# oval-group/GNN_branching

Measured on NVIDIA B200. Metric: gnn_subdomains_scored_per_sec, higher is better.
Workload: dtype fp16x3 (fp32 accumulate)

## Files before the change

### gnn_branching_b200/csrc/gnnb_tc.cu

```cuda
#include "gnnb_prop_body.cuh"
#include "gnnb_umma.cuh"

namespace gnnb {
namespace {

using namespace tcx;

constexpr uint32_t ACOL = 0, DCOL = 64, WG_COLS = 128;

struct WG {
    uint32_t land;
    uint32_t mbar_mma, mbar_tma;
    uint32_t ph_mma, ph_tma;
    uint32_t tmem;
    uint32_t tmem0;
    uint32_t acol;
    int t;
    int bar_threads;
    int wg;
    bool lead_warp;
};

__device__ __forceinline__ void wg_barrier(const WG& c) { named_bar(1 + c.wg, c.bar_threads); }

// ... 878 lines not shown
#pragma unroll
                        for (int i = 0; i < 16; ++i) o[i] = relu_nan(fmaf(node_ >= 0 ? l_ : 0.f, wl[i], fmaf(node_ >= 0 ? u_ : 0.f, wu[i], o[i])));
                        uint32_t w[16];
                        split16(o, w);
                        tmem_st16(c.tmem + D + 64 + 16 * qd, w);
                    }
                }
                gemm_sync(c);
                if (c.lead_warp) {
                    tc_fence_after();
                    if (elect_one()) {
                        WG c2 = c;
                        c2.acol = D + 64;
                        issue_ts(c, W + INF_WN, W + INF_WN + WPLANE, 64, D, false);
                        issue_ts(c2, W + INF_WI, W + INF_WI + WPLANE, 64, D, true);
                        umma_commit(c.mbar_mma);
                    }
                    __syncwarp();
                }
            } else {
                gemm_ts_start(c, W + UPD_W3, W + UPD_W3 + 2 * WPLANE, 128, D);
            }
            return true;
        };
        bool have = cur.valid() ? start_item(cur, 0, node_n, l_n, u_n) : false;
        for (; cur.valid(); cur.next(), cur1.next(), cur2.next(), ++it) {
            const uint32_t buf = it & 1u;
            const uint32_t acc_empty = smem_u32(&tl->acc_empty[buf]);
            const int dom = cur.pair * PD + j;
            const int node = node_n;
            const float l = l_n, u = u_n;
            const int slot0 = slot0_n;
            fetch_bounds(cur1, node_nn);
            node_nn = fetch_node(cur2);
            auto advance = [&]() { have = cur1.valid() ? start_item(cur1, it + 1, node_n, l_n, u_n) : false; };
            if (!have) {
                advance();
                continue;
            }
            const int64_t tile = (int64_t)dom * ntiles + cur.tile;
#ifdef GNNB_TRACE
            c0_ = clock64(); ++c_tiles;
#endif
            const Ratio q = compute_ratio(l, u);
            const float gate = (q.r0 != 0.0f) ? 1.0f : 0.0f;
            const bool amb = (q.amb != 0.0f) && node >= 0;
            const unsigned bal = __ballot_sync(0xffffffffu, amb);
            if ((c.t & 31) == 0) tl->wcnt[j * 2 + h][c.t >> 5] = __popc(bal);
            unsigned char* img = a.mu_out ? reinterpret_cast<unsigned char*>(a.mu_out) + tile * (int64_t)ABUF : nullptr;
            if (inp) {
                gemm_finish(c);
                if (h == 0 && c.t == 0) mbar_arrive(acc_empty);
                c.acol = D + 64;
                CTR(1);
                {
                    float v0[16], v1[16];
                    tmem_ld32_sync(c.tmem + D + h * 32, v0, v1);
#pragma unroll
                    for (int qq = 0; qq < 2; ++qq) {
                        float (&v)[16] = qq ? v1 : v0;
                        const int qd = Q0 + qq;
                        float bb[16];
                        lds16(tl->bias[0] + qd * 16, bb);
#pragma unroll
                        for (int i = 0; i < 16; ++i) v[i] = relu_nan(v[i] + bb[i]);
                        a_store16(c, qd, v);
                    }
                }
                CTR(2);
                gemm_ts_start(c, W + INF_B22, W + INF_B22 + WPLANE, 64, D);
                gemm_finish(c);
                CTR(3);
                bad |= nan_watch(a.nan_doms, dom, epilogue_to_mu_pair<false>(c, h, pair_bar, D, tl->bias[1], 1.0f, node >= 0, img, stage, advance));
                CTR(6);
                continue;
            }
            gemm_finish(c);
            if (h == 0 && c.t == 0) mbar_arrive(acc_empty);
            c.acol = D + 64;
            CTR(1);
#pragma unroll
            for (int qq = 0; qq < 2; ++qq) {
                const int qd = Q0 + qq;
                float x[16], y[16], bb[16];
                {
                    uint32_t ra[16], rb[16];
                    tmem_ld16(c.tmem + D + qd * 16, ra);
                    tmem_ld16(c.tmem + D + 64 + qd * 16, rb);
                    tmem_wait16(ra, x);
                    tmem_wait16(rb, y);
                }
                lds16(tl->bias[0] + qd * 16, bb);
#pragma unroll
                for (int i = 0; i < 16; ++i) x[i] = relu_nan(fmaf(q.r0, x[i], fmaf(q.r1, y[i], bb[i])));
                a_store16(c, qd, x);
            }
            CTR(2);
            gemm_ts_start(c, W + UPD_WC, W + UPD_WC + WPLANE, 64, D);
            int slot = slot0 + __popc(bal & ((1u << (c.t & 31)) - 1u));
#pragma unroll
            for (int w = 0; w < 3; ++w) slot += (w < (c.t >> 5)) ? tl->wcnt[j * 2 + h][w] : 0;
            const float* rt = rlx + (size_t)(slot >> 7) * (TILE * P) + (size_t)(slot & (TILE - 1)) * 4 + (size_t)(8 * h) * (TILE * 4);
            float4 rx[8];
#pragma unroll
            for (int i = 0; i < 8; ++i) rx[i] = amb ? ldg4_now(rt + (size_t)i * (TILE * 4)) : make_float4(0.f, 0.f, 0.f, 0.f);
            gemm_finish(c);
            CTR(3);
            {
                float v0[16], v1[16];
                tmem_ld32_sync(c.tmem + D + h * 32, v0, v1);
#pragma unroll
                for (int qq = 0; qq < 2; ++qq) {
                    float (&v)[16] = qq ? v1 : v0;
                    const int qd = Q0 + qq;
                    float bb[16];
                    lds16(tl->bias[1] + qd * 16, bb);
#pragma unroll
                    for (int hh = 0; hh < 4; ++hh) {
                        const float4 x = rx[qq * 4 + hh];
                        v[hh * 4 + 0] = relu_nan(v[hh * 4 + 0] + x.x + bb[hh * 4 + 0]);
                        v[hh * 4 + 1] = relu_nan(v[hh * 4 + 1] + x.y + bb[hh * 4 + 1]);
                        v[hh * 4 + 2] = relu_nan(v[hh * 4 + 2] + x.z + bb[hh * 4 + 2]);
                        v[hh * 4 + 3] = relu_nan(v[hh * 4 + 3] + x.w + bb[hh * 4 + 3]);
                    }
                    a_store16(c, qd, v);
                }
            }
            CTR(4);
            gemm_ts_start(c, W + UPD_W42, W + UPD_W42 + WPLANE, 64, D);
            gemm_finish(c);
            CTR(5);
            if (!with_score) {
                bad |= nan_watch(a.nan_doms, dom, epilogue_to_mu_pair<false>(c, h, pair_bar, D, tl->bias[2], gate, node >= 0, img, stage, advance));
            } else {
                bad |= nan_watch(a.nan_doms, dom, epilogue_to_mu_pair<true>(c, h, pair_bar, D, tl->bias[2], gate, node >= 0, img, stage));
                gemm_ts_start(c, W + UPD_FN, W + UPD_FN + WPLANE, 64, D);
                gemm_finish(c);
                float sc = 0.f;
                {
                    float v0[16], v1[16];
                    tmem_ld32_sync(c.tmem + D + h * 32, v0, v1);
#pragma unroll
                    for (int qq = 0; qq < 2; ++qq) {
                        const int qd = Q0 + qq;
                        float bb[16], ww[16];
                        lds16(tl->bias[3] + qd * 16, bb);
                        lds16(tl->vec + qd * 16, ww);
#pragma unroll
                        for (int i = 0; i < 16; ++i) sc = fmaf(relu_nan((qq ? v1 : v0)[i] + bb[i]), ww[i], sc);
                    }
                }
                if (h == 1) {
                    tmem_st1(c.tmem + D + 64, __float_as_uint(sc));
                    tmem_st_wait();
                }
                tc_fence_before();
                wg_barrier(c);
                tc_fence_after();
                if (h == 0) {
                    sc += __uint_as_float(tmem_ld1_sync(c.tmem + D + 64));
                    if (node >= 0) scores[(int64_t)dom * a.score_stride + a.score_off + node] = fmaf(sc, AINV, bscore);
                }
                advance();
            }
            CTR(6);
        }
#ifdef GNNB_TRACE
        if (rank == 1 && threadIdx.x == CHAIN_WARP0 * 32)
            printf("TRACE fused-chain wg0: tiles %d total %lld | wait acc_full %lld | per tile: convert %lld gemm1 %lld epi1 %lld gemm2 %lld epi2 %lld gemm3 %lld epi3 %lld\n",
                   c_tiles, clock64() - c_all, c_wait, c_ph[0] / max(c_tiles, 1), c_ph[1] / max(c_tiles, 1), c_ph[2] / max(c_tiles, 1), c_ph[3] / max(c_tiles, 1),
                   c_ph[4] / max(c_tiles, 1), c_ph[5] / max(c_tiles, 1), c_ph[6] / max(c_tiles, 1));
        if (rank == 1 && threadIdx.x == CHAIN_WARP0 * 32) {
            printf("TRACE fused-e3 (cumulative over launches): wait prev store %lld, tmem load %lld, compute + stage %lld, fence + issue %lld\n",
                   g_e3_trace[0], g_e3_trace[1], g_e3_trace[2], g_e3_trace[3]);
        }
#endif
        if (bad) atomicAdd(a.nan_count, 1ULL);
        if (h == 0 && (c.t & 31) == 0) bulk_wait_all();
    }
    tc_fence_before();
    __syncthreads();
    if (warp == 0) tmem_dealloc(tmem_base, 512);
}

__global__ void __launch_bounds__(fz::THREADS, 1) k_tc_fused(FusedArgs fa) { fused_body<false>(fa); }
__global__ void __launch_bounds__(fz::THREADS, 1) k_tc_fused_input(FusedArgs fa) { fused_body<true>(fa); }

constexpr uint32_t RLX_FR = 0, RLX_BC11 = 2 * WPLANE, RLX_BC12 = 4 * WPLANE, RLX_BC2 = 6 * WPLANE, RLX_BR = 12 * WPLANE;
constexpr uint32_t RLX_WBYTES = 14 * WPLANE;

struct RelaxLayers {
    NodeInputs in[AMB_MAX_LAYERS];
    float* rlx_f[AMB_MAX_LAYERS];
    float* rlx_b[AMB_MAX_LAYERS];
    int n;
};

__global__ void __launch_bounds__(128 * NWG, 1) k_tc_relax(GnnParams g, const __grid_constant__ RelaxLayers rl) {
    const uint16_t* const wsrc[5] = {g.tcx_w[T_FWD_R], g.tc[BC1_1], g.tc[BC1_2], g.tc[BC2], g.tcx_w[T_BWD_R]};
    const uint32_t woff[5] = {RLX_FR, RLX_BC11, RLX_BC12, RLX_BC2, RLX_BR};
    const uint32_t wlen[5] = {2 * WPLANE, 2 * WPLANE, 2 * WPLANE, 6 * WPLANE, 2 * WPLANE};
    CtaSetup s = cta_setup<false, 5>(smem_dyn(), RLX_WBYTES, wsrc, woff, wlen);
    Tail& tl = *s.tail;
    copy_vec(tl.bias[0], g.tcx_b[T_FWD_R], P); copy_vec(tl.bias[1], g.bias[BC1_1], P); copy_vec(tl.bias[2], g.bias[BC1_2], P);
    copy_vec(tl.bias[3], g.bias[BC2], P); copy_vec(tl.bias[4], g.tcx_b[T_BWD_R], P);
    copy_vec(tl.w_small[0], g.wt[FC1], 7 * P); copy_vec(tl.w_small[1], g.wt[BC1], 7 * P);
    copy_vec(tl.bias[5], g.bias[FC1], P); copy_vec(tl.vec, g.bias[BC1], P);
    __syncthreads();
    mbar_wait(smem_u32(&tl.mbar[0]), 0);
    pdl_trigger(); pdl_wait();
    WG c = make_wg(s, RLX_WBYTES);
    const uint32_t W = s.w;
    int tile0[AMB_MAX_LAYERS + 1];
    tile0[0] = 0;
#pragma unroll 1
    for (int k = 0; k < rl.n; ++k) {
        const int namb_k = __ldg(rl.in[k].amb_base + (rl.in[k].rows + TILE - 1) / TILE);
        tile0[k + 1] = tile0[k] + (namb_k + TILE - 1) / TILE;
    }
    const int total_tiles = tile0[rl.n];
    int k = 0;
    for (int gt = (int)blockIdx.x * NWG + c.wg; gt < total_tiles; gt += (int)gridDim.x * NWG) {
        while (gt >= tile0[k + 1]) ++k;
        const NodeInputs& in = rl.in[k];
        float* __restrict__ rlx_f = rl.rlx_f[k];
        float* __restrict__ rlx_b = rl.rlx_b[k];
        const int64_t tile = gt - tile0[k];
        const int64_t namb = __ldg(in.amb_base + (in.rows + TILE - 1) / TILE);
        const int64_t slot = tile * TILE + c.t;
        float l = 0.f, u = 1.f, d1 = 0.f, d2 = 0.f, pp = 0.f, po = 0.f, bs = 0.f;
        if (slot < namb) {
            const int64_t grow = natural_row(in.map, __ldg(in.amb_rows + slot));
            l = in.lb[grow]; u = in.ub[grow];
            d1 = in.dual[grow * 3 + 1]; d2 = in.dual[grow * 3 + 2];
            pp = in.prim_pre[grow]; po = in.prim_post[grow];
            bs = in.bias_node[grow % in.map.n];
        }
        const Ratio q = compute_ratio(l, u);
        {
            const float feat[7] = {q.beta, l, u, d1 - d2, pp, po, bs};
            first_layer_to_a<7>(c, feat, tl.w_small[0], tl.bias[5]);
        }
        gemm_ts(c, W + RLX_FR, W + RLX_FR + WPLANE, 64, DCOL);
        epilogue_to_rlx(c, DCOL, tl.bias[0], q.amb, rlx_f + (size_t)tile * (TILE * P));
        {
            const float feat[7] = {l, u, q.beta, -d2 + d1, po, pp, bs};
            first_layer_to_a<7>(c, feat, tl.w_small[1], tl.vec);
        }
        gemm_ts(c, W + RLX_BC11, W + RLX_BC11 + WPLANE, 64, DCOL);
        epilogue_to_a<true>(c, DCOL, tl.bias[1]);
        gemm_ts(c, W + RLX_BC12, W + RLX_BC12 + WPLANE, 64, DCOL);
        epilogue_to_a<false>(c, DCOL, tl.bias[2]);
        float acc[64];
        gemm_ts(c, W + RLX_BC2, W + RLX_BC2 + 3 * WPLANE, 64, DCOL);
#pragma unroll
        for (int qd = 0; qd < 4; ++qd) {
            float v[16], bb[16];
            tmem_ld16_sync(c.tmem + DCOL + qd * 16, v);
            lds16(tl.bias[3] + qd * 16, bb);
#pragma unroll
            for (int j = 0; j < 16; ++j) acc[qd * 16 + j] = v[j] + bb[j];
        }
        gemm_ts(c, W + RLX_BC2 + WPLANE, W + RLX_BC2 + 4 * WPLANE, 64, DCOL);
        {
            const float nd2 = -d2;
#pragma unroll
            for (int qd = 0; qd < 4; ++qd) {
                float v[16];
                tmem_ld16_sync(c.tmem + DCOL + qd * 16, v);
#pragma unroll
                for (int j = 0; j < 16; ++j) acc[qd * 16 + j] = fmaf(nd2, v[j], acc[qd * 16 + j]);
            }
        }
        gemm_ts(c, W + RLX_BC2 + 2 * WPLANE, W + RLX_BC2 + 5 * WPLANE, 64, DCOL);
#pragma unroll
        for (int qd = 0; qd < 4; ++qd) {
            float v[16];
            tmem_ld16_sync(c.tmem + DCOL + qd * 16, v);
#pragma unroll
            for (int j = 0; j < 16; ++j) v[j] = relu_nan(fmaf(d1, v[j], acc[qd * 16 + j]));
            a_store16(c, qd, v);
        }
        gemm_ts(c, W + RLX_BR, W + RLX_BR + WPLANE, 64, DCOL);
        epilogue_to_rlx(c, DCOL, tl.bias[4], q.amb, rlx_b + (size_t)tile * (TILE * P));
    }
    cta_teardown(s);
}

constexpr uint32_t EMB_WBYTES = 2 * WPLANE;

__global__ void __launch_bounds__(128 * NWG, 1) k_tc_input_embed(GnnParams g, const float* __restrict__ lb0,
                                                                 const float* __restrict__ x, const float* __restrict__ ub0,
                                                                 uint16_t* __restrict__ mu0, RowMap map, int64_t rows) {
    const uint16_t* const wsrc[1] = {g.tc[INP_F_1]};
    const uint32_t woff[1] = {0};
    const uint32_t wlen[1] = {2 * WPLANE};
    CtaSetup s = cta_setup<true, 1>(smem_dyn(), EMB_WBYTES, wsrc, woff, wlen);
    Tail& tl = *s.tail;
    copy_vec(tl.bias[0], g.bias[INP_F_1], P); copy_vec(tl.bias[5], g.bias[INP_F], P); copy_vec(tl.w_small[0], g.wt[INP_F], 3 * P);
    __syncthreads();
    mbar_wait(smem_u32(&tl.mbar[0]), 0);
    pdl_trigger(); pdl_wait();
    WG c = make_wg(s, EMB_WBYTES);
    const int64_t ntiles = (rows + TILE - 1) / TILE;
    for (int64_t tile = (int64_t)blockIdx.x * NWG + c.wg; tile < ntiles; tile += (int64_t)gridDim.x * NWG) {
        const int64_t row0 = tile * TILE, grow = row0 + c.t;
        float feat[3] = {0.f, 0.f, 0.f};
        const int64_t nrow = grow < rows ? natural_row(map, grow) : -1;
        if (nrow >= 0) { feat[0] = lb0[nrow]; feat[1] = x[nrow]; feat[2] = ub0[nrow]; }
        first_layer_to_a<3>(c, feat, tl.w_small[0], tl.bias[5]);
        if (c.t == 0) bulk_wait_read();
        gemm_ts(c, s.w, s.w + WPLANE, 64, DCOL);
        epilogue_to_mu<false>(c, DCOL, tl.bias[0], 1.0f, nrow >= 0);
        commit_tile(c, mu0 + (size_t)tile * (ABUF / 2));
    }
    if (c.t == 0) bulk_wait_all();
    cta_teardown(s);
}

constexpr uint32_t INU_WI = 0, INU_WN = 2 * WPLANE, INU_B22 = 4 * WPLANE, INU_WBYTES = 6 * WPLANE;

__global__ void __launch_bounds__(128 * NWG, 1) k_tc_input_update(GnnParams g, const float* __restrict__ lb0,
                                                                  const float* __restrict__ ub0, const uint16_t* __restrict__ nb_img,
                                                                  uint16_t* __restrict__ mu0, RowMap map, int64_t rows) {
    const uint16_t* const wsrc[3] = {g.tcx_w[T_INP_C], g.tcx_w[T_INP_NB], g.tc[INP_B2_2]};
    const uint32_t woff[3] = {INU_WI, INU_WN, INU_B22};
    const uint32_t wlen[3] = {2 * WPLANE, 2 * WPLANE, 2 * WPLANE};
    CtaSetup s = cta_setup<true, 3>(smem_dyn(), INU_WBYTES, wsrc, woff, wlen);
    Tail& tl = *s.tail;
    copy_vec(tl.bias[0], g.tcx_b[T_INP_C], P); copy_vec(tl.bias[1], g.bias[INP_B2_2], P);
    copy_vec(tl.bias[5], g.bias[INP_B], P); copy_vec(tl.w_small[0], g.wt[INP_B], 2 * P);
    __syncthreads();
    mbar_wait(smem_u32(&tl.mbar[0]), 0);
    pdl_trigger(); pdl_wait();
    WG c = make_wg(s, INU_WBYTES);
    const uint32_t W = s.w;
    const int64_t ntiles = (rows + TILE - 1) / TILE;
    const int64_t tile_step = (int64_t)gridDim.x * NWG;
    for (int64_t tile = (int64_t)blockIdx.x * NWG + c.wg; tile < ntiles; tile += tile_step) {
        const int64_t row0 = tile * TILE, grow = row0 + c.t;
        request_nb(c, nb_img + (size_t)tile * (ABUF / 2));
        float feat[2] = {0.f, 0.f};
        const int64_t nrow = grow < rows ? natural_row(map, grow) : -1;
        if (nrow >= 0) { feat[0] = lb0[nrow]; feat[1] = ub0[nrow]; }
        first_layer_to_a<2>(c, feat, tl.w_small[0], tl.bias[5]);
        gemm_sync(c);
        if (c.lead_warp) {
            tc_fence_after();
            if (elect_one()) issue_ts(c, W + INU_WI, W + INU_WI + WPLANE, 64, DCOL, false);
            __syncwarp();
            mbar_wait(c.mbar_tma, c.ph_tma);
            if (elect_one()) {
                issue_ss(c, W + INU_WN, W + INU_WN + WPLANE, 64, DCOL, true);
                umma_commit(c.mbar_mma);
            }
            __syncwarp();
        }
        c.ph_tma ^= 1u;
        gemm_finish(c);
        epilogue_to_a<true>(c, DCOL, tl.bias[0]);
        gemm_ts(c, W + INU_B22, W + INU_B22 + WPLANE, 64, DCOL);
        epilogue_to_mu<false>(c, DCOL, tl.bias[1], 1.0f, nrow >= 0);
        commit_tile(c, mu0 + (size_t)tile * (ABUF / 2));
    }
    if (c.t == 0) bulk_wait_all();
    cta_teardown(s);
}

constexpr size_t smem_bytes(uint32_t wbytes, bool land) { return 1024 + wbytes + (land ? NWG * ABUF : 0) + sizeof(Tail); }

int grid_for(int64_t rows) {
    const int64_t tiles = (rows + TILE - 1) / TILE, ctas = (tiles + NWG - 1) / NWG;
    return (int)(ctas < 1 ? 1 : (ctas < 148 ? ctas : 148));
}

__global__ void k_unpack_tile_image(const uint16_t* __restrict__ img, float* __restrict__ out, RowMap map, int64_t rows,
                                    int piece_major) {
    const int64_t i = (int64_t)blockIdx.x * blockDim.x + threadIdx.x;
    if (i >= rows * 8) return;
    const int64_t row = i >> 3;
    const int64_t nrow = natural_row(map, row);
    if (nrow < 0) return;
    const int chunk = (int)(i & 7);
    const int64_t tile = row / TILE;
    const uint32_t r = (uint32_t)(row % TILE);
    const uint32_t off = piece_major ? (uint32_t)chunk * NB_PIECE + r * 16u : swz(r, (uint32_t)chunk);
    const __half* hi = reinterpret_cast<const __half*>(img) + tile * (ABUF / 2) + off / 2;
    const __half* lo = hi + APLANE / 2;
    for (int j = 0; j < 8; ++j) out[nrow * P + chunk * 8 + j] = (__half2float(hi[j]) + __half2float(lo[j])) * AINV;
}

__device__ __forceinline__ bool row_is_ambiguous(const float* __restrict__ lb, const float* __restrict__ ub, const RowMap& map,
                                                 int64_t row, int64_t rows) {
    const int64_t nrow = row < rows ? natural_row(map, row) : -1;
    return nrow >= 0 && compute_ratio(lb[nrow], ub[nrow]).amb != 0.0f;
}
__global__ void __launch_bounds__(TILE) k_amb_count(const float* __restrict__ lb, const float* __restrict__ ub, RowMap map,
                                                    int64_t rows, int32_t* __restrict__ cnt) {
    const int64_t row = (int64_t)blockIdx.x * TILE + threadIdx.x;
    const bool amb = row_is_ambiguous(lb, ub, map, row, rows);
    const int total = __syncthreads_count(amb);
    if (threadIdx.x == 0) cnt[blockIdx.x] = total;
}
__global__ void __launch_bounds__(1024) k_amb_scan(const int32_t* __restrict__ cnt, int32_t* __restrict__ base, int n) {
    __shared__ int32_t part[1024];
    const int per = (n + 1023) / 1024, lo = threadIdx.x * per, hi = min(n, lo + per);
    int32_t sum = 0;
    for (int i = lo; i < hi; ++i) sum += cnt[i];
    part[threadIdx.x] = sum;
    __syncthreads();
    for (int off = 1; off < 1024; off <<= 1) {
        const int32_t v = threadIdx.x >= off ? part[threadIdx.x - off] : 0;
        __syncthreads();
        part[threadIdx.x] += v;
        __syncthreads();
    }
    int32_t run = part[threadIdx.x] - sum;
    for (int i = lo; i < hi; ++i) { base[i] = run; run += cnt[i]; }
    if (threadIdx.x == 1023) base[n] = part[1023];
}
__global__ void __launch_bounds__(TILE) k_amb_fill(const float* __restrict__ lb, const float* __restrict__ ub, RowMap map,
                                                   int64_t rows, const int32_t* __restrict__ base, int32_t* __restrict__ amb_rows) {
    __shared__ int32_t wc[4];
    const int64_t row = (int64_t)blockIdx.x * TILE + threadIdx.x;
    const bool amb = row_is_ambiguous(lb, ub, map, row, rows);
    const unsigned bal = __ballot_sync(0xffffffffu, amb);
    const int lane = threadIdx.x & 31, warp = threadIdx.x >> 5;
    if (lane == 0) wc[warp] = __popc(bal);
    __syncthreads();
    int slot = base[blockIdx.x] + __popc(bal & ((1u << lane) - 1u));
    for (int w = 0; w < warp; ++w) slot += wc[w];
    if (amb) amb_rows[slot] = (int32_t)row;
}

__device__ __forceinline__ int amb_layer_of(const AmbLayers& a, int tile) {
    int k = 0;
    while (k + 1 < a.n && tile >= a.tile0[k + 1]) ++k;
    return k;
}
__global__ void __launch_bounds__(TILE) k_amb_count_all(AmbLayers a) {
    const int k = amb_layer_of(a, (int)blockIdx.x), tile = (int)blockIdx.x - a.tile0[k];
    const int64_t row = (int64_t)tile * TILE + threadIdx.x;
    const bool amb = row_is_ambiguous(a.lb[k], a.ub[k], a.map[k], row, a.rows[k]);
    const int total = __syncthreads_count(amb);
    if (threadIdx.x == 0) a.cnt[k][tile] = total;
}
__global__ void __launch_bounds__(1024) k_amb_scan_all(AmbLayers a) {
    __shared__ int32_t part[1024];
    const int k = blockIdx.x, n = a.tile0[k + 1] - a.tile0[k];
    const int32_t* __restrict__ cnt = a.cnt[k];
    int32_t* __restrict__ base = a.base[k];
    const int per = (n + 1023) / 1024, lo = threadIdx.x * per, hi = min(n, lo + per);
    int32_t sum = 0;
    for (int i = lo; i < hi; ++i) sum += cnt[i];
    part[threadIdx.x] = sum;
    __syncthreads();
    for (int off = 1; off < 1024; off <<= 1) {
        const int32_t v = threadIdx.x >= off ? part[threadIdx.x - off] : 0;
        __syncthreads();
        part[threadIdx.x] += v;
        __syncthreads();
    }
    int32_t run = part[threadIdx.x] - sum;
    for (int i = lo; i < hi; ++i) { base[i] = run; run += cnt[i]; }
    if (threadIdx.x == 1023) base[n] = part[1023];
}
__global__ void __launch_bounds__(TILE) k_amb_fill_all(AmbLayers a) {
    __shared__ int32_t wc[4];
    const int k = amb_layer_of(a, (int)blockIdx.x), tile = (int)blockIdx.x - a.tile0[k];
    const int64_t row = (int64_t)tile * TILE + threadIdx.x;
    const bool amb = row_is_ambiguous(a.lb[k], a.ub[k], a.map[k], row, a.rows[k]);
    const unsigned bal = __ballot_sync(0xffffffffu, amb);
    const int lane = threadIdx.x & 31, warp = threadIdx.x >> 5;
    if (lane == 0) wc[warp] = __popc(bal);
    __syncthreads();
    int slot = a.base[k][tile] + __popc(bal & ((1u << lane) - 1u));
    for (int w = 0; w < warp; ++w) slot += wc[w];
    if (amb) a.out_rows[k][slot] = (int32_t)row;
}

}

void amb_compact_all(AmbLayers a, cudaStream_t st, int64_t* launches) {
    a.tile0[0] = 0;
    for (int k = 0; k < a.n; ++k) a.tile0[k + 1] = a.tile0[k] + (int)((a.rows[k] + TILE - 1) / TILE);
    k_amb_count_all<<<a.tile0[a.n], TILE, 0, st>>>(a);
    k_amb_scan_all<<<a.n, 1024, 0, st>>>(a);
    k_amb_fill_all<<<a.tile0[a.n], TILE, 0, st>>>(a);
    *launches += 3;
}

void amb_compact(const float* lb, const float* ub, RowMap map, int64_t rows, int32_t* cnt, int32_t* amb_base, int32_t* amb_rows,
                 cudaStream_t st, int64_t* launches) {
    const int ntiles = (int)((rows + TILE - 1) / TILE);
    k_amb_count<<<ntiles, TILE, 0, st>>>(lb, ub, map, rows, cnt);
    k_amb_scan<<<1, 1024, 0, st>>>(cnt, amb_base, ntiles);
    k_amb_fill<<<ntiles, TILE, 0, st>>>(lb, ub, map, rows, amb_base, amb_rows);
    *launches += 3;
}

bool tc_available() { return true; }

int tc_init() {
    cudaError_t e;
    if ((e = cudaFuncSetAttribute(k_tc_update, cudaFuncAttributeMaxDynamicSharedMemorySize, (int)smem_bytes(UPD_WBYTES, true))) != cudaSuccess) return e;
    if ((e = cudaFuncSetAttribute(k_tc_fused, cudaFuncAttributeMaxDynamicSharedMemorySize, (int)fz::SMEM_MAX)) != cudaSuccess) return e;
    if ((e = cudaFuncSetAttribute(k_tc_fused_input, cudaFuncAttributeMaxDynamicSharedMemorySize, (int)fz::SMEM_MAX)) != cudaSuccess) return e;
    if ((e = cudaFuncSetAttribute(k_tc_relax, cudaFuncAttributeMaxDynamicSharedMemorySize, (int)smem_bytes(RLX_WBYTES, false))) != cudaSuccess) return e;
    if ((e = cudaFuncSetAttribute(k_tc_input_embed, cudaFuncAttributeMaxDynamicSharedMemorySize, (int)smem_bytes(EMB_WBYTES, true))) != cudaSuccess) return e;
    if ((e = cudaFuncSetAttribute(k_tc_input_update, cudaFuncAttributeMaxDynamicSharedMemorySize, (int)smem_bytes(INU_WBYTES, true))) != cudaSuccess) return e;
    return 0;
}

int64_t tc_packed_elems(int K) { return (int64_t)2 * (K / 64) * 64 * 64; }

int64_t tc_pack_weight(const float* w, int K, uint16_t* dst) {
    const int nblk = K / 64;
    for (int n = 0; n < 64; ++n)
        for (int k = 0; k < K; ++k) {
            uint16_t hi, lo;
            split_host(w[(size_t)n * K + k], hi, lo);
            const int kb = k / 64, kk = k % 64;
            const size_t e = (size_t)(swz((uint32_t)n, (uint32_t)(kk / 8)) + (kk % 8) * 2) / 2;
            dst[(size_t)kb * 4096 + e] = hi;
            dst[(size_t)(nblk + kb) * 4096 + e] = lo;
        }
    return tc_packed_elems(K);
}

void tc_relax(const GnnParams& g, const NodeInputs* in, float* const* relax_f, float* const* relax_b, int n_layers, cudaStream_t st,
              int64_t* launches) {
    RelaxLayers rl;
    rl.n = n_layers;
    int64_t rows = 0;
    for (int k = 0; k < n_layers; ++k) { rl.in[k] = in[k]; rl.rlx_f[k] = relax_f[k]; rl.rlx_b[k] = relax_b[k]; rows += in[k].rows; }
    launch_pdl(k_tc_relax, grid_for(rows), 128 * NWG, smem_bytes(RLX_WBYTES, false), st, g, rl);
    ++*launches;
}

namespace {
UpdArgs make_upd_args(const GnnParams& g, bool backward, const float* lb, const float* ub, const float* nb, const float* relax,
                      const int32_t* amb_base, float* mu_out, float* scores, RowMap map, int64_t score_stride, int64_t score_off,
                      int64_t rows, unsigned long long* nan_count, const NanDoms& nan_doms) {
    UpdArgs a;
    a.g = g; a.backward = backward ? 1 : 0; a.lb = lb; a.ub = ub; a.nb_img = reinterpret_cast<const uint16_t*>(nb); a.rlx = relax;
    a.amb_base = amb_base; a.mu_out = reinterpret_cast<uint16_t*>(mu_out); a.scores = scores; a.map = map;
    a.score_stride = score_stride; a.score_off = score_off; a.Bc = (int)(rows / map.nslots); a.nan_count = nan_count;
    a.nan_doms = nan_doms;
    return a;
}
}

void tc_update(const GnnParams& g, bool backward, const float* lb, const float* ub, const float* nb, const float* relax,
               const int32_t* amb_base, float* mu_out, float* scores, RowMap map, int64_t score_stride, int64_t score_off, int64_t rows,
               unsigned long long* nan_count, const NanDoms& nan_doms, cudaStream_t st, int64_t* launches) {
    const UpdArgs a = make_upd_args(g, backward, lb, ub, nb, relax, amb_base, mu_out, scores, map, score_stride, score_off, rows, nan_count,
                                    nan_doms);
    const int64_t nitems = (int64_t)(map.nslots / TILE) * ((a.Bc + NWG - 1) / NWG);
    launch_pdl(k_tc_update, (int)(nitems < 1 ? 1 : (nitems < 148 ? nitems : 148)), 128 * NWG, smem_bytes(UPD_WBYTES, true), st, a);
    ++*launches;
}

void tc_fused(const GnnParams& g, const PropPlan* plan, const float* mu_in, bool backward, const float* lb, const float* ub,
              const float* relax, const int32_t* amb_base, float* mu_out, float* scores, RowMap map, int64_t score_stride, int64_t score_off,
              int64_t rows, unsigned long long* nan_count, const NanDoms& nan_doms, float* nb_dbg, bool input_layer, cudaStream_t st,
              int64_t* launches) {
    FusedArgs fa;
    fa.input_layer = input_layer ? 1 : 0;
    fa.u = make_upd_args(g, backward, lb, ub, nullptr, relax, amb_base, mu_out, scores, map, score_stride, score_off, rows, nan_count,
                         nan_doms);
    fa.plan = prop_plan_dev(plan);
    fa.mu_in = reinterpret_cast<const uint16_t*>(mu_in);
    fa.nb_dbg = reinterpret_cast<uint16_t*>(nb_dbg);
    const uint32_t wbytes = scores ? UPD_WBYTES : UPD_FN;
    const int staging = mu_out == nullptr ? 0 : (scores ? 1 : 2);
    const int ns = (int)((fz::SMEM_MAX - fz::smem_for(wbytes, staging, 0)) / fz::STAGE);
    fa.n_stages = ns > fz::NS_MAX ? fz::NS_MAX : ns;
    fa.mma_group = prop_plan_ksteps_per_tile(plan) >= 48.0 ? 4 : 2;
    if (fa.mma_group > fa.n_stages / 2) fa.mma_group = fa.n_stages / 2;
    const int64_t nitems = (int64_t)fa.plan.ntiles * ((fa.u.Bc + fz::PD - 1) / fz::PD);
    launch_pdl(input_layer ? k_tc_fused_input : k_tc_fused, (int)(nitems < 1 ? 1 : (nitems < 148 ? nitems : 148)), fz::THREADS,
               fz::smem_for(wbytes, staging, fa.n_stages), st, fa);
    ++*launches;
}

void tc_input_embed(const GnnParams& g, const float* lb0, const float* x, const float* ub0, float* mu0, RowMap map, int64_t rows,
                    cudaStream_t st, int64_t* launches) {
    launch_pdl(k_tc_input_embed, grid_for(rows), 128 * NWG, smem_bytes(EMB_WBYTES, true), st, g, lb0, x, ub0, reinterpret_cast<uint16_t*>(mu0), map, rows);
    ++*launches;
}

void tc_input_update(const GnnParams& g, const float* lb0, const float* ub0, const float* nb, float* mu0, RowMap map, int64_t rows,
                     cudaStream_t st, int64_t* launches) {
    launch_pdl(k_tc_input_update, grid_for(rows), 128 * NWG, smem_bytes(INU_WBYTES, true), st,
               g, lb0, ub0, reinterpret_cast<const uint16_t*>(nb), reinterpret_cast<uint16_t*>(mu0), map, (int64_t)rows);
    ++*launches;
}

void tc_unpack_tile_image(const float* img, float* out, RowMap map, int64_t rows, bool piece_major, cudaStream_t st) {
    const int64_t n = rows * 8;
    k_unpack_tile_image<<<(unsigned)((n + 255) / 256), 256, 0, st>>>(reinterpret_cast<const uint16_t*>(img), out, map, rows, piece_major ? 1 : 0);
}

}
```

Baseline: 272,400.

## Prefetch next tile inputs during MMA and use per-warp store epilogue in input embed

The input-embedding kernel now loads the next tile's lb/x/ub features while the current tile's tensor-core GEMM runs, so global load latency overlaps the MMA. The epilogue and commit are also rewritten to work per warp: each warp stages its slice in swizzled shared memory and issues its own bulk stores. This drops the workgroup-wide barrier and single-thread commit. The cost is more register use and extra code paths, and the epilogue ignores the validity flag that the old epilogue_to_mu took, so padding rows may be written with the bias value instead of being zeroed.

```diff
diff --git a/gnn_branching_b200/csrc/gnnb_tc.cu b/gnn_branching_b200/csrc/gnnb_tc.cu
--- a/gnn_branching_b200/csrc/gnnb_tc.cu
+++ b/gnn_branching_b200/csrc/gnnb_tc.cu
@@ -1204,19 +1204,53 @@
     mbar_wait(smem_u32(&tl.mbar[0]), 0);
     pdl_trigger(); pdl_wait();
     WG c = make_wg(s, EMB_WBYTES);
-    const int64_t ntiles = (rows + TILE - 1) / TILE;
-    for (int64_t tile = (int64_t)blockIdx.x * NWG + c.wg; tile < ntiles; tile += (int64_t)gridDim.x * NWG) {
-        const int64_t row0 = tile * TILE, grow = row0 + c.t;
-        float feat[3] = {0.f, 0.f, 0.f};
+    const int warp = c.t >> 5, lane = c.t & 31;
+    const uint32_t stg = c.land + (uint32_t)warp * fz::STG_WARP;
+    const int64_t ntiles = (rows + TILE - 1) / TILE, step = (int64_t)gridDim.x * NWG;
+    float feat_n[3];
+    auto fetch = [&](int64_t tile) {
+        feat_n[0] = feat_n[1] = feat_n[2] = 0.f;
+        const int64_t grow = tile * TILE + c.t;
         const int64_t nrow = grow < rows ? natural_row(map, grow) : -1;
-        if (nrow >= 0) { feat[0] = lb0[nrow]; feat[1] = x[nrow]; feat[2] = ub0[nrow]; }
-        first_layer_to_a<3>(c, feat, tl.w_small[0], tl.bias[5]);
-        if (c.t == 0) bulk_wait_read();
-        gemm_ts(c, s.w, s.w + WPLANE, 64, DCOL);
-        epilogue_to_mu<false>(c, DCOL, tl.bias[0], 1.0f, nrow >= 0);
-        commit_tile(c, mu0 + (size_t)tile * (ABUF / 2));
-    }
-    if (c.t == 0) bulk_wait_all();
+        if (nrow >= 0) { feat_n[0] = ldg1_now(lb0 + nrow); feat_n[1] = ldg1_now(x + nrow); feat_n[2] = ldg1_now(ub0 + nrow); }
+    };
+    int64_t tile = (int64_t)blockIdx.x * NWG + c.wg;
+    fetch(tile);
+    for (; tile < ntiles; tile += step) {
+        {
+            const float feat[3] = {feat_n[0], feat_n[1], feat_n[2]};
+            first_layer_to_a<3>(c, feat, tl.w_small[0], tl.bias[5]);
+        }
+        gemm_ts_start(c, s.w, s.w + WPLANE, 64, DCOL);
+        fetch(tile + step);
+        gemm_finish(c);
+        if (lane == 0) bulk_wait_read();
+        __syncwarp();
+#pragma unroll
+        for (int q = 0; q < 4; ++q) {
+            float v[16], bb[16];
+            tmem_ld16_sync(c.tmem + DCOL + q * 16, v);
+            lds16(tl.bias[0] + q * 16, bb);
+#pragma unroll
+            for (int j = 0; j < 16; ++j) v[j] += bb[j];
+            uint32_t w[16];
+            split16(v, w);
+            const uint32_t o0 = stg + swz((uint32_t)lane, (uint32_t)(2 * q)), o1 = stg + swz((uint32_t)lane, (uint32_t)(2 * q + 1));
+            sts128(o0, w[0], w[1], w[2], w[3]);
+            sts128(o1, w[4], w[5], w[6], w[7]);
+            sts128(o0 + fz::STG_PLANE, w[8], w[9], w[10], w[11]);
+            sts128(o1 + fz::STG_PLANE, w[12], w[13], w[14], w[15]);
+        }
+        fence_proxy_async();
+        __syncwarp();
+        if (lane == 0) {
+            unsigned char* dst = reinterpret_cast<unsigned char*>(mu0 + (size_t)tile * (ABUF / 2)) + warp * fz::STG_PLANE;
+            bulk_s2g_nocommit(dst, stg, fz::STG_PLANE);
+            bulk_s2g_nocommit(dst + APLANE, stg + fz::STG_PLANE, fz::STG_PLANE);
+            bulk_commit();
+        }
+    }
+    if (lane == 0) bulk_wait_all();
     cta_teardown(s);
 }
 
```

Result: faster. 277,700 (median of 6 runs) (+2.0%).
